# theislab/dca

Hardware: NVIDIA H100
Metric: cells/sec (ZINB AE epoch, device-timed) (higher is better)
Workload: dtype bf16-gemm/f32-acc/f32-loss

## Files before the change

dca_b200/csrc/dca_internal.cuh:

```cuda
#pragma once
#include <cuda_runtime.h>
#include <cuda_bf16.h>
#include <stdint.h>
#include <stddef.h>
#include <atomic>
#include "../../include/dca_b200.h"

namespace dca {

void set_error(const char* fmt, ...);
extern std::atomic<long long> g_launches;
inline void count_launch(int n = 1) { g_launches.fetch_add(n, std::memory_order_relaxed); }

#define DCA_CUDA_OK(expr)                                                              \
  do {                                                                                 \
    cudaError_t _e = (expr);                                                           \
    if (_e != cudaSuccess) {                                                           \
      ::dca::set_error("%s failed: %s (%s:%d)", #expr, cudaGetErrorString(_e), __FILE__, __LINE__); \
      return DCA_ERR_CUDA;                                                             \
    }                                                                                  \
  } while (0)

#define DCA_LAUNCH_CHECK()                                                             \
  do {                                                                                 \
// ... 42 lines not shown
int bn_train_finalize(const double* sum, const double* sq, int M, int N, float eps, float momentum,
                      float* mean, float* inv_std, float* moving_mean, float* moving_var, cudaStream_t s);
int bn_relu_fwd(const float* a, int64_t ld, int M, int N, const float* mean, const float* inv_std,
                const float* beta, float* xhat, float* h, __nv_bfloat16* h_bf16, cudaStream_t s);
int bn_infer_prepare(const float* moving_mean, const float* moving_var, int N, float eps,
                     float* mean, float* inv_std, cudaStream_t s);
int bias_relu_fwd(const float* a, int64_t ld, int M, int N, float* h, __nv_bfloat16* h_bf16, cudaStream_t s);
int relu_bwd(float* dh, const float* h, int64_t ld, int M, int N, cudaStream_t s);
int bn_bwd_apply(float* g_inout, const float* xhat, int64_t ld, int M, int N, const float* inv_std,
                 const double* sum_g, const double* sum_gx, float* dbeta, cudaStream_t s, int stat_rows = 0);
int col_sum_to_float(const double* sum, int N, float* out, cudaStream_t s);
int theta_prepare(const float* theta_raw, int G, float* theta, float* chain, cudaStream_t s);
int theta_grad_finish(const float* dtheta, const float* chain, int G, float scale, float* grad_out, cudaStream_t s);
int add_reg_grad(const float* w, float* g, int64_t n, float l1, float l2, cudaStream_t s);
int reg_penalty(const float* w, int64_t n, float l1, float l2, double* acc, cudaStream_t s);
int rmsprop_update(float* params, const float* grads, float* rms, int64_t n, float lr, float clip,
                   float rho, float eps, float grad_scale, __nv_bfloat16* shadow, float* loss_out, cudaStream_t s);
struct OptScalars { int kind; float lr, clip, gs, c0, c1, c2, c3, c4; };
int optimizer_update(float* params, const float* grads, float* s1, float* s2, int64_t n, OptScalars o, __nv_bfloat16* shadow,
                     float* loss_out, cudaStream_t s);
int glorot_fill(float* w, int64_t n, int fan_in, int fan_out, uint64_t seed, uint64_t stream_id, cudaStream_t s);
int fill_value(float* p, int64_t n, float v, cudaStream_t s);
int cast_to_bf16(const float* in, __nv_bfloat16* out, int64_t n, cudaStream_t s);

__device__ __forceinline__ float pre_log_value(float y, double sf64, int flags) {
  float q = (flags & DCA_PRE_SIZE_FACTORS) ? (float)((double)y / sf64) : y;
  if ((flags & DCA_PRE_LOG1P) && q != 0.f) q = (float)log1p((double)q);
  return q;
}
struct ExactXform {
  const double* n_counts; double median; int flags;
  const double* mean; const double* std; const float* x_zero;
};
int exact_zero_inputs(const double* mean, const double* std, int n, float* x_zero, cudaStream_t s);
int expand_counts(const void* cnt, int bits, const float* sf_in, int M, int n, const float* mean, const float* inv_std, int use_sf,
                  int use_log1p, float* Yout, void* Xout, int x_bf16, float* sf_out, const int64_t* ovf_indptr,
                  const void* ovf_entries, cudaStream_t s, const ExactXform* ex = nullptr, const int32_t* rows = nullptr);
int expand_sparse(const void* bitmap, const int64_t* nib_indptr, const void* nibbles, const float* sf_in, int M, int n,
                  const float* mean, const float* inv_std, int use_sf, int use_log1p, float* Yout, void* Xout, int x_bf16,
                  float* sf_out, const int64_t* ovf_indptr, const void* ovf_entries, int max_row_nibble_bytes, cudaStream_t s,
                  const ExactXform* ex = nullptr, const int32_t* rows = nullptr);
int check_packed_counts(const char* who, const dca_packed_counts* p);
int gather_rows_bf16(const void* X, int x_bf16, int64_t ldx, const int32_t* rows, int M, int n, __nv_bfloat16* out,
                     cudaStream_t s);

namespace tc {
int heads_fwd_tc(const __nv_bfloat16* Hb, int B, const __nv_bfloat16* const W[3], const float* const bias[3], int G,
                 int n_heads, const int kind[3], const float* row_scale, float* const out[3], int64_t ld_out, int sm_count,
                 cudaStream_t s);
int gene_gemm_tc(int mode, const __nv_bfloat16* const Z[3], int64_t ldz, const int32_t* rows, int B, int G, int n_heads,
                 const __nv_bfloat16* H, const __nv_bfloat16* const W[3], float* out_b, float* const dW[3], int64_t dW_ld,
                 int dW_transposed, float* const db[3], void* ws, size_t ws_bytes, int sm_count, cudaStream_t s);
size_t gene_gemm_workspace_bytes(int B);
int flash_zinb_tc(const __nv_bfloat16* H3, int B, int G, const __nv_bfloat16* const W[3], const float* const bias[3],
                  const float* Y, int64_t ldy, const int32_t* rows, const float* sf, float ridge, float inv_n,
                  float* dH3, float* const dW[3], float* const db[3], void* ws, size_t ws_bytes, double* loss_sum,
                  const double* penalty, float* loss_slot, double* epoch_acc, int batch, const float* lf_dev, int sm_count,
                  cudaStream_t s);
}

struct LossArgs {
  const float* Y; int64_t ldy; const int32_t* rows; const float* sf;
  const float* m; const float* d; const float* pi; int64_t ld;
  int B, G; int ae_type; float ridge; float inv_n;
  void* dzm; void* dzd; void* dzp; int grad_bf16;
  float* dtheta;
  double* loss_sum;
  void* ws; size_t ws_bytes;
  int counter_ready = 0;
  float* fin_loss_slot = nullptr; double* fin_epoch_acc = nullptr; const double* fin_penalty = nullptr; int fin_batch = 0;
};
size_t loss_workspace_bytes(int B, int G);
extern int g_fused_heads_default;
const float* loss_log_fact_table();
int zinb_loss_fwd_bwd(const LossArgs& a, cudaStream_t s);
int zinb_loss_fwd(const LossArgs& a, cudaStream_t s);

struct HeadsLossArgs {
  const __nv_bfloat16* H3; int B, G;
  const __nv_bfloat16* W[3]; const float* bias[3];
  const float* Y; int64_t ldy; const int32_t* rows; const float* sf;
  float ridge, inv_n;
  __nv_bfloat16* dz[3]; int64_t ldz;
  double* loss_sum; void* ws; size_t ws_bytes;
  int counter_ready = 0;
  float* fin_loss_slot = nullptr; double* fin_epoch_acc = nullptr; const double* fin_penalty = nullptr; int fin_batch = 0;
};
int heads_loss_tc(const HeadsLossArgs& a, cudaStream_t s);

}
```

dca_b200/csrc/engine.cu:

```cuda
#include <cmath>
#include <cstdarg>
#include <cstdio>
#include <cstring>
#include <cstdlib>
#include <string>
#include <vector>
#include "dca_internal.cuh"
#include "engine.h"

namespace dca {

std::atomic<long long> g_launches{0};
static thread_local char g_err[512] = "";

void set_error(const char* fmt, ...) {
  va_list ap;
  va_start(ap, fmt);
  vsnprintf(g_err, sizeof(g_err), fmt, ap);
  va_end(ap);
}

namespace {

inline size_t align_up(size_t v, size_t a = 256) { return (v + a - 1) / a * a; }
// ... 190 lines not shown
    cudaEvent_t e;
    if (cudaEventCreate(&e) != cudaSuccess) return;
    prof.ev.push_back(e); prof.phase.push_back(-1);
  }
  prof.phase[prof.n] = phase;
  cudaEventRecord(prof.ev[prof.n], s);
  ++prof.n;
}

int Engine::prof_collect() {
  if (prof.n == 0) return DCA_OK;
  DCA_CUDA_OK(cudaEventSynchronize(prof.ev[prof.n - 1]));
  for (size_t i = 0; i + 1 < prof.n; ++i) {
    const int ph = prof.phase[i];
    if (ph < 0 || ph >= DCA_N_PHASES) continue;
    float ms = 0.f;
    if (cudaEventElapsedTime(&ms, prof.ev[i], prof.ev[i + 1]) == cudaSuccess) { prof.ms[ph] += ms; prof.cnt[ph] += 1; }
  }
  prof.n = 0;
  return DCA_OK;
}

void Engine::bind(void* base_) {
  base = reinterpret_cast<char*>(base_);
}

int Engine::gemm_auto(GemmArgs g, cudaStream_t s) {
  const long long tiles = (long long)cdiv(g.M, 64) * cdiv(g.N, 64), target = 2ll * sm_count;
  int splits = 1;
  if (g.epilogue == EPI_ACCUM && tiles < target && g.K >= 256) {
    splits = (int)((target + tiles - 1) / tiles);
    const int maxs = g.K / 128;
    if (splits > maxs) splits = maxs;
    if (splits < 1) splits = 1;
  }
  g.splits = splits;
  return gemm_generic(g, s);
}

int Engine::forward(const void* X, int64_t ldx, const int32_t* rows, int Bn, bool training, cudaStream_t s) {
  const void* hin = X; int64_t ldin = ldx; int in_bf16 = x_override_bf16 ? 1 : (cfg.x_dtype == DCA_BF16); const int32_t* gather = rows;
  cur_x = XOperand{};
  if (tc_enc && (reinterpret_cast<uintptr_t>(X) & 15) == 0) {
    if (in_bf16 && ldx % 8 == 0) cur_x = XOperand{reinterpret_cast<const __nv_bfloat16*>(X), ldx, rows};
    else if (!in_bf16 && ldx % 4 == 0) {
      DCA_TRY(gather_rows_bf16(X, in_bf16, ldx, rows, Bn, cfg.n_in, bf(o_xb), s));
      cur_x = XOperand{bf(o_xb), cfg.n_in, nullptr};
    }
  }
  const bool fused = use_mid(Bn);
  for (int i = 0; i < (fused ? 1 : L); ++i) {
    Layer& l = lay[i];
    float* a = f(l.o_a);
    DCA_TRY(fill_rows_with_bias(a, l.out, Bn, l.out, pp(l.b), s));
    if (i == 0 && cur_x.base) {
      const __nv_bfloat16* Z[3] = {cur_x.base, cur_x.base, cur_x.base};
      const __nv_bfloat16* W1[3] = {bf(o_pbf) + lay[0].W, bf(o_pbf) + lay[0].W, bf(o_pbf) + lay[0].W};
      DCA_TRY(tc::gene_gemm_tc(1, Z, cur_x.ld, cur_x.rows, Bn, cfg.n_in, 1, nullptr, W1, a, nullptr, 0, 0, nullptr, base + o_ggws, ggws_bytes, sm_count, s));
    } else {
    GemmArgs g{};
    g.A = hin; g.lda = ldin; g.a_bf16 = in_bf16; g.transA = 0; g.a_rows = gather;
    g.B = pp(l.W); g.ldb = l.out; g.transB = 0;
    g.C = a; g.ldc = l.out; g.M = Bn; g.N = l.out; g.K = l.in; g.epilogue = EPI_ACCUM;
    DCA_TRY(gemm_auto(g, s));
    }
    if (fused) break;
    if (cfg.batchnorm) {
      if (training) {
        DCA_TRY(col_sums(a, nullptr, l.out, Bn, l.out, d(o_dsum), d(o_dprod), d(o_scratch), s));
        DCA_TRY(bn_allreduce(d(o_dsum), d(o_dprod), l.out, s));
        DCA_TRY(bn_train_finalize(d(o_dsum), d(o_dprod), bn_rows(Bn), l.out, cfg.bn_eps, cfg.bn_momentum, f(l.o_mean),
                                  f(l.o_inv), st(l.mm), st(l.mv), s));
      } else {
        DCA_TRY(bn_infer_prepare(st(l.mm), st(l.mv), l.out, cfg.bn_eps, f(l.o_mean), f(l.o_inv), s));
      }
    }
    DCA_TRY(act_fwd(l, Bn, training, (tc_heads && i == L - 1) ? bf(o_h3b) : nullptr, s));
    hin = f(l.o_h); ldin = l.out; in_bf16 = 0; gather = nullptr;
  }
  if (fused) {
    mid::Params mp;
    mid_params(mp, Bn, training);
    DCA_TRY(mid_forward(mp, s));
    hin = f(lay[L - 1].o_h); ldin = lay[L - 1].out; in_bf16 = 0; gather = nullptr;
  }
  head_in = hin; head_ld = ldin; head_bf16 = in_bf16; head_rows = gather;
  return DCA_OK;
}

int Engine::x_gather_sf(const float* sf, const int32_t* rows, int Bn, cudaStream_t s) {
  gather_sf_kernel<<<cdiv(Bn, 256), 256, 0, s>>>(sf, rows, Bn, f(o_sfb));
  DCA_LAUNCH_CHECK();
  return DCA_OK;
}

void Engine::mid_params(mid::Params& p, int Bn, bool training) {
  memset(&p, 0, sizeof(p));
  p.L = L; p.B = Bn; p.training = training ? 1 : 0; p.batchnorm = cfg.batchnorm; p.center = L / 2;
  for (int i = 0; i < L; ++i) {
    Layer& l = lay[i];
    p.w[i] = l.out; p.W[i] = pp(l.W); p.b[i] = pp(l.b);
    p.beta[i] = cfg.batchnorm ? pp(l.beta) : nullptr;
    p.mm[i] = cfg.batchnorm ? st(l.mm) : nullptr; p.mv[i] = cfg.batchnorm ? st(l.mv) : nullptr;
    p.mean[i] = f(l.o_mean); p.inv[i] = f(l.o_inv); p.xhat[i] = f(l.o_xhat); p.h[i] = f(l.o_h);
    p.gW[i] = gp(l.W); p.gb[i] = gp(l.b); p.gbeta[i] = cfg.batchnorm ? gp(l.beta) : nullptr;
  }
  p.a0 = f(lay[0].o_a); p.a_center = f(lay[L / 2].o_a);
  p.h_last_bf16 = tc_heads ? bf(o_h3b) : nullptr;
  p.partial = d(o_midpart); p.gpart = f(o_midgpart); p.bar = reinterpret_cast<unsigned*>(base + o_bar);
  p.eps = cfg.bn_eps; p.momentum = cfg.bn_momentum;
}

int Engine::heads_forward(int Bn, float* m_out, float* d_out, float* p_out, int64_t ld_out, const float* row_scale,
                          cudaStream_t s) {
  const int G = cfg.n_out;
  if (tc_heads && (ld_out % 4 == 0)) {
    float* outs_by_head[3] = {m_out, d_out, p_out};
    bool all = true;
    for (int k = 0; k < n_slots; ++k) all = all && outs_by_head[slot_head[k]] && ((reinterpret_cast<uintptr_t>(outs_by_head[slot_head[k]]) & 15) == 0);
    if (all) {
      float* outs[3] = {nullptr, nullptr, nullptr};
      for (int k = 0; k < n_slots; ++k) outs[k] = outs_by_head[slot_head[k]];
      for (int k = n_slots; k < 3; ++k) outs[k] = outs[0];
      const __nv_bfloat16* Wk[3]; const float* bk[3];
      for (int k = 0; k < 3; ++k) { const int kk = k < n_slots ? k : 0; Wk[k] = bf(o_pbf) + head_W[slot_head[kk]]; bk[k] = pp(head_b[slot_head[kk]]); }
      return tc::heads_fwd_tc(bf(o_h3b), Bn, Wk, bk, G, n_slots, slot_kind, row_scale, outs, ld_out, sm_count, s);
    }
  }
  struct H { int k; float* out; int epi; const float* rs; } hs[3] = {
      {0, m_out, EPI_MEAN_ACT, row_scale}, {1, d_out, EPI_DISP_ACT, nullptr}, {2, p_out, EPI_SIGMOID, nullptr}};
  for (auto& h : hs) {
    if (head_W[h.k] < 0 || !h.out) continue;
    GemmArgs g{};
    g.A = head_in; g.lda = head_ld; g.a_bf16 = head_bf16; g.transA = 0; g.a_rows = head_rows;
    g.B = pp(head_W[h.k]); g.ldb = G; g.transB = 0;
// ... 1094 lines not shown
```

dca_b200/csrc/gene_gemm_tc.cu:

```cuda
#include "engine.h"
#include "tc_common.cuh"

namespace dca {
namespace tc {
int g_gg_profile = 0;
int g_head_bwd_banded = 1;
int g_head_bwd_stagger = 1300;
namespace gg {

constexpr int kThreads = 256;
constexpr uint32_t kZBytes = 128 * 128 * 2;
constexpr uint32_t kWBytes = 64 * 128 * 2;
constexpr uint32_t kHBytes = 128 * 64 * 2;
constexpr uint32_t kOutBytes = 128 * 64 * 4;
constexpr uint32_t kOnesBytes = 16 * 128;
constexpr int kMaxGb = 4;
constexpr int kMaxSlots = 16;

static_assert(kWBytes == kHBytes, "the two item kinds of the banded launch share one stage shape");
template <bool DO_A, bool DO_B, bool BANDED>
constexpr int stages() { return DO_A && DO_B && !BANDED ? 2 : 3; }
template <bool DO_A, bool DO_B, bool BANDED>
constexpr uint32_t stage_bytes() { return BANDED ? kZBytes + kWBytes : kZBytes + (DO_B ? kWBytes : 0) + (DO_A ? kHBytes : 0); }
template <bool DO_A, bool DO_B, bool COLSUM, bool BANDED>
constexpr uint32_t smem_bytes() {
  return stages<DO_A, DO_B, BANDED>() * stage_bytes<DO_A, DO_B, BANDED>() + (DO_A ? kOutBytes : 0) + (COLSUM ? kOnesBytes : 0) + 1024;
}

struct BandItem { int kind, head, gr, gb0, ng, cb0, ncb; };

__host__ __device__ inline BandItem band_item(int k, int n_gb, int n_cb, int gpr, int ranges) {
  const int per_head = n_gb + ranges * n_cb, full_band = gpr + n_cb;
  BandItem it;
  it.head = k / per_head; k -= it.head * per_head;
  it.gr = min(k / full_band, ranges - 1); k -= it.gr * full_band;
  const int gb0 = it.gr * gpr, ng = min(n_gb, gb0 + gpr) - gb0, m = min(ng, n_cb);
  int idx;
  if (k < 2 * m) { it.kind = k & 1; idx = k >> 1; }
  else { it.kind = ng > n_cb ? 0 : 1; idx = k - m; }
  if (it.kind == 0) { it.gb0 = gb0 + idx; it.ng = 1; it.cb0 = 0; it.ncb = n_cb; }
  else { it.gb0 = gb0; it.ng = ng; it.cb0 = idx; it.ncb = 1; }
  return it;
}

struct Params {
  int B, G, n_heads;
  int n_cb, n_gb;
  int gb_per_item, cb_per_item;
  int gene_ranges, cell_splits;
  int total_items;
  int stagger;
  float* db[3];
  float* part; int64_t part_stride;
  const int32_t* rows; const __nv_bfloat16* zsrc; int64_t ldz;
};

__device__ __forceinline__ void cp_async_16(uint32_t smem_dst, const void* src, uint32_t src_bytes) {
  asm volatile("cp.async.cg.shared.global [%0], [%1], 16, %2;" ::"r"(smem_dst), "l"(src), "r"(src_bytes) : "memory");
}
__device__ __forceinline__ void cp_async_commit() { asm volatile("cp.async.commit_group;" ::: "memory"); }
template <int N>
__device__ __forceinline__ void cp_async_wait() { asm volatile("cp.async.wait_group %0;" ::"n"(N) : "memory"); }

template <bool DO_A, bool DO_B, bool COLSUM, bool WK, int MAXG, bool BANDED>
__global__ void __launch_bounds__(kThreads, 1)
gene_gemm_kernel(const __grid_constant__ CUtensorMap map_z0, const __grid_constant__ CUtensorMap map_z1,
                 const __grid_constant__ CUtensorMap map_z2, const __grid_constant__ CUtensorMap map_h,
                 const __grid_constant__ CUtensorMap map_w0, const __grid_constant__ CUtensorMap map_w1,
                 const __grid_constant__ CUtensorMap map_w2, const __grid_constant__ CUtensorMap map_dw0, const __grid_constant__ CUtensorMap map_dw1,
                 const __grid_constant__ CUtensorMap map_dw2, const int dw_transposed, const Params p) {
  static_assert(!BANDED || (DO_A && DO_B && MAXG == 1), "banded items hold one gene block of (a) accumulators");
  constexpr int kStages = stages<DO_A, DO_B, BANDED>();
  constexpr uint32_t kStage = stage_bytes<DO_A, DO_B, BANDED>();
  constexpr uint32_t kHOff = kZBytes + (DO_B && !BANDED ? kWBytes : 0);
  extern __shared__ __align__(1024) uint8_t smem_raw[];
  uint8_t* smem = smem_raw + ((1024u - (smem_u32(smem_raw) & 1023u)) & 1023u);
  uint8_t* s_st = smem;
  float* s_o = reinterpret_cast<float*>(s_st + kStages * kStage);
  uint8_t* s_ones = reinterpret_cast<uint8_t*>(s_o) + (DO_A ? kOutBytes : 0);
  __shared__ uint64_t full[kStages];

  if (threadIdx.x == 0) {
    for (int i = 0; i < kStages; ++i) mbar_init(&full[i], 1);
    fence_barrier_init();
  }
  if (COLSUM) {
    for (int i = threadIdx.x; i < (int)kOnesBytes / 4; i += kThreads) reinterpret_cast<uint32_t*>(s_ones)[i] = 0x3F803F80u;
    fence_proxy_async_smem();
  }
  __syncthreads();

  const int wg = threadIdx.x >> 7, w = (threadIdx.x >> 5) & 3, l = threadIdx.x & 31;
  const int frow = 16 * w + (l >> 2), fcol = 2 * (l & 3);

  auto stage_begin = [&]() {
    if (threadIdx.x == 0) bulk_wait_read<0>();
    __syncthreads();
  };
  auto stage_end = [&](const CUtensorMap* m, int c0, int c1) {
    fence_proxy_async_smem();
    __syncthreads();
    if (threadIdx.x == 0) { tma_reduce_add_2d(m, c0, c1, s_o); bulk_commit(); }
  };

  uint32_t T0 = 0;
  const bool gather = p.rows != nullptr;
  const int g_rh = threadIdx.x >> 3, g_c = threadIdx.x & 7, g_h = g_rh & 1, g_r0 = g_rh >> 1;
  const uint32_t g_dst = g_h * (kZBytes / 2) + g_r0 * 128 + ((g_c ^ (g_r0 & 7)) << 4);
  int src_row[8];
  if constexpr (BANDED) {
    if (p.stagger > 0 && blockIdx.x < p.total_items) {
      const BandItem it = band_item(blockIdx.x, p.n_gb, p.n_cb, p.gb_per_item, p.gene_ranges);
      const long long wait = (long long)(it.kind ? it.cb0 : it.gb0 - it.gr * p.gb_per_item) * p.stagger;
      if (threadIdx.x == 0) {
        const long long c0 = clock64();
        while (clock64() - c0 < wait) __nanosleep(100);
      }
      __syncthreads();
    }
  }
  for (int item = blockIdx.x; item < p.total_items; item += gridDim.x) {
    int head, gr, gb0, ng, cb0, ncb;
    bool ia = DO_A, ib = DO_B;
    if constexpr (BANDED) {
      const BandItem it = band_item(item, p.n_gb, p.n_cb, p.gb_per_item, p.gene_ranges);
// ... 162 lines not shown
            const int g = gb * 128 + wg * 64 + frow;
            if (g < p.G) atomicAdd(dbh + g, acc_c[j][0]);
            if (g + 8 < p.G) atomicAdd(dbh + g + 8, acc_c[j][2]);
          }
        }
      }
    }
  }
  if (threadIdx.x == 0) bulk_wait<0>();
}

__global__ void gene_gemm_reduce_kernel(const float* __restrict__ part, int slots, int64_t stride, float* __restrict__ out,
                                        int64_t n) {
  const int64_t i = ((int64_t)blockIdx.x * blockDim.x + threadIdx.x) * 4;
  if (i >= n) return;
  float4 acc = *reinterpret_cast<const float4*>(out + i);
  for (int sl = 0; sl < slots; ++sl) {
    const float4 v = __ldcs(reinterpret_cast<const float4*>(part + sl * stride + i));
    acc.x += v.x; acc.y += v.y; acc.z += v.z; acc.w += v.w;
  }
  *reinterpret_cast<float4*>(out + i) = acc;
}

void plan_a(Params& p, int n_heads, int sm_count) {
  int best_gpi = 1; long long best_cost = -1;
  for (int gpi = 1; gpi <= kMaxGb; ++gpi) {
    const long long items = (long long)cdiv(p.n_gb, gpi) * n_heads, rounds = (items + sm_count - 1) / sm_count;
    const long long cost = rounds * ((long long)gpi * p.n_cb + 2ll * gpi);
    if (best_cost < 0 || cost < best_cost) { best_cost = cost; best_gpi = gpi; }
  }
  p.gb_per_item = best_gpi; p.gene_ranges = cdiv(p.n_gb, best_gpi);
  p.cb_per_item = p.n_cb; p.cell_splits = 1;
  p.total_items = p.gene_ranges * n_heads;
}
void plan_b(Params& p, int n_heads, int sm_count) {
  p.cb_per_item = 1; p.cell_splits = p.n_cb;
  int gsplits = cdiv(4 * sm_count, p.n_cb * n_heads); if (gsplits < 1) gsplits = 1;
  if (gsplits > kMaxSlots / n_heads) gsplits = kMaxSlots / n_heads;
  if (gsplits > p.n_gb) gsplits = p.n_gb;
  while (gsplits > 1 && cdiv(p.n_gb, gsplits) < 4) --gsplits;
  p.gb_per_item = cdiv(p.n_gb, gsplits); p.gene_ranges = cdiv(p.n_gb, p.gb_per_item);
  p.total_items = p.gene_ranges * p.cell_splits * n_heads;
}
void plan_banded(Params& p, int n_heads, int sm_count, int* grid) {
  plan_b(p, n_heads, sm_count);
  p.total_items = n_heads * (p.n_gb + p.gene_ranges * p.n_cb);
  const int band = p.gb_per_item + p.n_cb;
  *grid = min(p.total_items, sm_count >= band ? sm_count / band * band : sm_count);
}

}

size_t gene_gemm_workspace_bytes(int B) { return sizeof(float) * (size_t)gg::kMaxSlots * cdiv(B, 128) * 128 * 64; }

int gene_gemm_tc(int mode, const __nv_bfloat16* const Z[3], int64_t ldz, const int32_t* rows, int B, int G, int n_heads,
                 const __nv_bfloat16* H, const __nv_bfloat16* const W[3], float* out_b, float* const dW[3], int64_t dW_ld,
                 int dW_transposed, float* const db[3], void* ws, size_t ws_bytes, int sm_count, cudaStream_t s) {
  using namespace gg;
  if (ldz % 8 != 0) { set_error("gene_gemm_tc: ldz must be a multiple of 8 (16-byte TMA stride)"); return DCA_ERR_BAD_ARG; }
  if (mode < 1 || mode > 3) { set_error("gene_gemm_tc: bad mode %d", mode); return DCA_ERR_BAD_ARG; }
  if (rows && (mode == 3 || n_heads != 1)) { set_error("gene_gemm_tc: row indices are for modes 1 and 2 (one Z)"); return DCA_ERR_BAD_ARG; }
  const bool do_a = mode & 2, do_b = mode & 1;
  if (do_b && (!ws || ws_bytes < gene_gemm_workspace_bytes(B))) { set_error("gene_gemm_tc: workspace too small"); return DCA_ERR_BAD_ARG; }
  CUtensorMap mz[3], mh, mw[3], mdw[3];
  for (int i = 0; i < 3; ++i) DCA_TRY(make_tensor_map_2d(&mz[i], Z[i < n_heads ? i : 0], 2, 1, (uint64_t)B, (uint64_t)G, (uint64_t)ldz, 128, 64, 1));
  mh = mz[0];
  for (int i = 0; i < 3; ++i) mw[i] = mdw[i] = mz[0];
  if (do_a) {
    DCA_TRY(make_tensor_map_2d(&mh, H, 2, 1, (uint64_t)B, 64, 64, 128, 64, 1));
    for (int i = 0; i < 3; ++i) {
      float* d = dW[i < n_heads ? i : 0];
      if (dW_transposed) DCA_TRY(make_tensor_map_2d(&mdw[i], d, 4, 0, 64, (uint64_t)G, (uint64_t)dW_ld, 64, 128, 0));
      else {
        if (dW_ld != 64) { set_error("gene_gemm_tc: non-transposed dW needs ld == 64"); return DCA_ERR_BAD_ARG; }
        DCA_TRY(make_tensor_map_2d(&mdw[i], d, 4, 0, (uint64_t)G, 64, 64, 128, 64, 0));
      }
    }
  }
  if (do_b) {
    for (int i = 0; i < 3; ++i) {
      const __nv_bfloat16* w = W[i < n_heads ? i : 0];
      if (mode == 3) DCA_TRY(make_tensor_map_2d(&mw[i], w, 2, 1, 64, (uint64_t)G, (uint64_t)G, 64, 64, 1));
      else DCA_TRY(make_tensor_map_2d(&mw[i], w, 2, 1, (uint64_t)G, 64, 64, 128, 64, 1));
    }
  }
  Params base{};
  base.B = B; base.G = G; base.n_heads = n_heads;
  base.n_cb = cdiv(B, 128); base.n_gb = cdiv(G, 128);
  for (int i = 0; i < 3; ++i) base.db[i] = db ? db[i] : nullptr;
  base.part = reinterpret_cast<float*>(ws); base.part_stride = (int64_t)base.n_cb * 128 * 64;
  base.rows = rows; base.zsrc = Z[0]; base.ldz = ldz;

#define DCA_GG_LAUNCH(P, GRID, A, Bb, Cc, WKk, MG, BND)                                                                \
  do {                                                                                                                 \
    static bool attr = false;                                                                                          \
    constexpr uint32_t sm = smem_bytes<A, Bb, Cc, BND>();                                                              \
    if (!attr) { DCA_CUDA_OK(cudaFuncSetAttribute(gene_gemm_kernel<A, Bb, Cc, WKk, MG, BND>, cudaFuncAttributeMaxDynamicSharedMemorySize, (int)sm)); attr = true; } \
    gene_gemm_kernel<A, Bb, Cc, WKk, MG, BND><<<GRID, kThreads, sm, s>>>(mz[0], mz[1], mz[2], mh, mw[0], mw[1], mw[2],  \
                                                                          mdw[0], mdw[1], mdw[2], dW_transposed, P);  \
    DCA_LAUNCH_CHECK();                                                                                                \
  } while (0)

  if (mode == 3 && g_head_bwd_banded) {
    Params p = base;
    int grid = 0;
    plan_banded(p, n_heads, sm_count, &grid);
    p.stagger = g_head_bwd_stagger;
    DCA_GG_LAUNCH(p, grid, true, true, true, true, 1, true);
    const int64_t n = (int64_t)B * 64;
    gene_gemm_reduce_kernel<<<(unsigned)cdiv(n / 4, 256), 256, 0, s>>>(p.part, p.gene_ranges * n_heads, p.part_stride, out_b, n);
    DCA_LAUNCH_CHECK();
    return DCA_OK;
  }
  if (do_a) {
    Params p = base;
    plan_a(p, n_heads, sm_count);
    const int grid = min(p.total_items, sm_count);
    if (mode == 3) DCA_GG_LAUNCH(p, grid, true, false, true, false, kMaxGb, false);
    else DCA_GG_LAUNCH(p, grid, true, false, false, false, kMaxGb, false);
  }
  if (do_b) {
    Params p = base;
    plan_b(p, n_heads, sm_count);
    const int grid = min(p.total_items, sm_count);
    if (mode == 3) DCA_GG_LAUNCH(p, grid, false, true, false, true, 1, false);
    else DCA_GG_LAUNCH(p, grid, false, true, false, false, 1, false);
    const int64_t n = (int64_t)B * 64;
    gene_gemm_reduce_kernel<<<(unsigned)cdiv(n / 4, 256), 256, 0, s>>>(p.part, p.gene_ranges * n_heads, p.part_stride, out_b, n);
    DCA_LAUNCH_CHECK();
  }
#undef DCA_GG_LAUNCH
  return DCA_OK;
}

}
}

using namespace dca;
extern "C" int dca_tc_gene_gemm_rows(int32_t mode, const void* Z0, const void* Z1, const void* Z2, int64_t ldz,
                                     const int32_t* rows, int32_t batch, int32_t genes, int32_t n_heads, const void* H,
                                     const void* W, float* out_b, float* dW0, float* dW1, float* dW2, int64_t dW_ld,
                                     int32_t dW_transposed, float* db0, float* db1, float* db2, void* stream, int32_t sm_count) {
  if (!Z0 || batch <= 0 || genes <= 0 || n_heads < 1 || n_heads > 3) { set_error("dca_tc_gene_gemm: bad argument"); return DCA_ERR_BAD_ARG; }
  int dev = 0, sms = 132;
  cudaGetDevice(&dev);
  cudaDeviceGetAttribute(&sms, cudaDevAttrMultiProcessorCount, dev);
  if (sm_count > 0 && sm_count < sms) sms = sm_count;
  const __nv_bfloat16* Z[3] = {(const __nv_bfloat16*)Z0, (const __nv_bfloat16*)Z1, (const __nv_bfloat16*)Z2};
  float* dW[3] = {dW0, dW1, dW2};
  float* db[3] = {db0, db1, db2};
  const __nv_bfloat16* Wp[3];
  for (int i = 0; i < 3; ++i) Wp[i] = (const __nv_bfloat16*)W + (mode == 3 ? (size_t)(i < n_heads ? i : 0) * 64 * genes : 0);
  cudaStream_t st = (cudaStream_t)stream;
  const size_t ws_bytes = tc::gene_gemm_workspace_bytes(batch);
  void* ws = nullptr;
  DCA_CUDA_OK(cudaMallocAsync(&ws, ws_bytes, st));
  const int rc = tc::gene_gemm_tc(mode, Z, ldz, rows, batch, genes, n_heads, (const __nv_bfloat16*)H, Wp, out_b, dW,
                                  dW_ld, dW_transposed, db, ws, ws_bytes, sms, st);
  DCA_CUDA_OK(cudaFreeAsync(ws, st));
  return rc;
}
extern "C" int dca_tc_gene_gemm_sms(int32_t mode, const void* Z0, const void* Z1, const void* Z2, int64_t ldz,
                                    int32_t batch, int32_t genes, int32_t n_heads, const void* H, const void* W, float* out_b,
                                    float* dW0, float* dW1, float* dW2, int64_t dW_ld, int32_t dW_transposed, float* db0,
                                    float* db1, float* db2, void* stream, int32_t sm_count) {
  return dca_tc_gene_gemm_rows(mode, Z0, Z1, Z2, ldz, nullptr, batch, genes, n_heads, H, W, out_b, dW0, dW1, dW2, dW_ld,
                               dW_transposed, db0, db1, db2, stream, sm_count);
}
extern "C" int dca_tc_gene_gemm(int32_t mode, const void* Z0, const void* Z1, const void* Z2, int64_t ldz, int32_t batch,
                                int32_t genes, int32_t n_heads, const void* H, const void* W, float* out_b, float* dW0,
                                float* dW1, float* dW2, int64_t dW_ld, int32_t dW_transposed, float* db0, float* db1,
                                float* db2, void* stream) {
  return dca_tc_gene_gemm_sms(mode, Z0, Z1, Z2, ldz, batch, genes, n_heads, H, W, out_b, dW0, dW1, dW2, dW_ld,
                              dW_transposed, db0, db1, db2, stream, 0);
}
extern "C" int dca_head_bwd_schedule(int32_t batch, int32_t genes, int32_t n_heads, int32_t sm_count, int32_t banded,
                                     int32_t* items, int64_t cap, int64_t* n_items, int32_t* grid) {
  if (batch <= 0 || genes <= 0 || n_heads < 1 || n_heads > 3 || sm_count < 1 || !n_items || !grid) {
    set_error("dca_head_bwd_schedule: bad argument"); return DCA_ERR_BAD_ARG;
// ... 38 lines not shown
```

dca_b200/csrc/mid_stack.cu:

```cuda
#include "dca_internal.cuh"
#include "mid_stack.h"
#include <cstdio>
#include <cstdlib>

namespace dca {
namespace mid {

constexpr int kThreads = 256;
#define MID_STAMP(i) do { if (p.dbg && blockIdx.x == 0 && threadIdx.x == 0) p.dbg[i] = clock64(); } while (0)
constexpr int kGenWord = 32;
constexpr int kStripStride = kMaxW + 4;
typedef float Strip[kStripStride];
typedef float WRow[kMaxW + 1];

__device__ __forceinline__ void grid_barrier(unsigned* bar, unsigned n, unsigned& gen) {
  __syncthreads();
  if (threadIdx.x == 0) {
    asm volatile("fence.acq_rel.gpu;" ::: "memory");
    const unsigned arrived = atomicAdd(&bar[0], 1u);
    if (arrived == n - 1) {
      bar[0] = 0;
      asm volatile("fence.acq_rel.gpu;" ::: "memory");
      atomicAdd(&bar[kGenWord], 1u);
    } else {
// ... 60 lines not shown
    for (int i = 0; i < kPairsPerWarp; ++i) tot[warp + i * (kThreads / 32)] = x[i][0];
  }
  __syncthreads();
}

__device__ __forceinline__ void strip_gemm(Strip* in, WRow* Ws, const float* bias, int rows, int w_in, int w_out, Strip* out) {
  const int c = threadIdx.x & 63, g = threadIdx.x >> 6;
  if (c < w_out) {
    const float bv = bias ? bias[c] : 0.f;
    for (int r0 = g * 4; r0 < rows; r0 += 16) {
      float acc[4] = {0.f, 0.f, 0.f, 0.f};
#pragma unroll 4
      for (int k = 0; k < w_in; k += 4) {
        const float w0 = Ws[k][c], w1 = Ws[k + 1][c], w2 = Ws[k + 2][c], w3 = Ws[k + 3][c];
#pragma unroll
        for (int j = 0; j < 4; ++j) {
          const float4 x = *reinterpret_cast<const float4*>(&in[r0 + j][k]);
          acc[j] = fmaf(x.x, w0, fmaf(x.y, w1, fmaf(x.z, w2, fmaf(x.w, w3, acc[j]))));
        }
      }
#pragma unroll
      for (int j = 0; j < 4; ++j)
        if (r0 + j < rows) out[r0 + j][c] = acc[j] + bv;
    }
  }
}

constexpr size_t kStripFloats = (size_t)(kMaxRows + 4) * kStripStride;
constexpr size_t kWsFloats = (size_t)kMaxW * (kMaxW + 1);
constexpr int kWSlots = DCA_MAX_HIDDEN - 1;
constexpr size_t kSmemBytes = sizeof(double) * (8 * kMaxW + 2 * kMaxW) + sizeof(float) * (2 * kStripFloats + kWSlots * kWsFloats + 2 * kMaxW) + 16;

__global__ void __launch_bounds__(kThreads, 1) mid_forward_kernel(const Params p) {
  extern __shared__ __align__(16) unsigned char smem_mid[];
  double (*red)[kMaxW] = reinterpret_cast<double (*)[kMaxW]>(smem_mid);
  double* tot = reinterpret_cast<double*>(smem_mid) + 8 * kMaxW;
  float* fbase = reinterpret_cast<float*>(tot + 2 * kMaxW);
  Strip* cur = reinterpret_cast<Strip*>(fbase);
  Strip* nxt = reinterpret_cast<Strip*>(fbase + kStripFloats);
  WRow* Ws = reinterpret_cast<WRow*>(fbase + 2 * kStripFloats);
  float* s_mean = fbase + 2 * kStripFloats + kWSlots * kWsFloats;
  float* s_inv = s_mean + kMaxW;
  __shared__ unsigned s_gen;
  if (threadIdx.x == 0) s_gen = *reinterpret_cast<volatile unsigned*>(&p.bar[kGenWord]);
  __syncthreads();
  unsigned gen = s_gen;
  MID_STAMP(0);

  const int row0 = blockIdx.x * p.rows_per_cta;
  const int rows = max(0, min(p.rows_per_cta, p.B - row0));
  for (int i = threadIdx.x; i < (int)kStripFloats; i += kThreads) { (&cur[0][0])[i] = 0.f; (&nxt[0][0])[i] = 0.f; }
  __syncthreads();
  const int tc = threadIdx.x & 63, tr = threadIdx.x >> 6;
  constexpr int kRowIters = kMaxRows / 4, kKIters = kMaxW / 4;
  float a0r[kRowIters];
#pragma unroll
  for (int i = 0; i < kRowIters; ++i) {
    const int r = tr + 4 * i;
    a0r[i] = (tc < p.w[0] && r < rows) ? p.a0[(size_t)(row0 + r) * p.w[0] + tc] : 0.f;
  }
  for (int l0 = 1; l0 < p.L; l0 += 2) {
    float wr[2][kKIters];
#pragma unroll
    for (int d = 0; d < 2; ++d) {
      const int l = l0 + d;
      const int win = l < p.L ? p.w[l - 1] : 0, w = l < p.L ? p.w[l] : 0;
#pragma unroll
      for (int i = 0; i < kKIters; ++i) { const int k = tr + 4 * i; wr[d][i] = (k < win && tc < w) ? p.W[l][(size_t)k * w + tc] : 0.f; }
    }
#pragma unroll
    for (int d = 0; d < 2; ++d) {
      if (l0 + d >= p.L) break;
      WRow* Wl = Ws + (size_t)(l0 + d - 1) * kMaxW;
#pragma unroll
      for (int i = 0; i < kKIters; ++i) Wl[tr + 4 * i][tc] = wr[d][i];
    }
  }
  float mm_old[DCA_MAX_HIDDEN], mv_old[DCA_MAX_HIDDEN];
#pragma unroll
  for (int l = 0; l < DCA_MAX_HIDDEN; ++l) {
    const bool mine = p.batchnorm && p.training && blockIdx.x == 0 && l < p.L && (int)threadIdx.x < p.w[l];
    mm_old[l] = mine ? p.mm[l][threadIdx.x] : 0.f; mv_old[l] = mine ? p.mv[l][threadIdx.x] : 0.f;
  }
  float beta_r[DCA_MAX_HIDDEN];
#pragma unroll
  for (int l = 0; l < DCA_MAX_HIDDEN; ++l) beta_r[l] = (p.batchnorm && l < p.L && tc < p.w[l]) ? p.beta[l][tc] : 0.f;
  if (tc < p.w[0]) {
#pragma unroll
    for (int i = 0; i < kRowIters; ++i) { const int r = tr + 4 * i; if (r < rows) cur[r][tc] = a0r[i]; }
  }
  __syncthreads();
  MID_STAMP(1);
  Strip* a = cur;
  Strip* o = nxt;
  for (int l = 0; l < p.L; ++l) {
    const int w = p.w[l];
    if (l > 0) {
      const int win = p.w[l - 1];
      strip_gemm(a, Ws + (size_t)(l - 1) * kMaxW, p.b[l], rows, win, w, o);
      __syncthreads();
      Strip* t = a; a = o; o = t;
      MID_STAMP(2 + l * 5);
    }
    if (l == p.center && p.a_center && !(l == 0 && p.a_center == p.a0) && tc < w)
      for (int r = tr; r < rows; r += 4) p.a_center[(size_t)(row0 + r) * w + tc] = a[r][tc];
    if (p.batchnorm) {
      if (p.training) {
        double* part = p.partial + (size_t)(l & 1) * kMaxCtas * 2 * kMaxW;
        cta_col_sums(a, a, rows, w, part + blockIdx.x, red);
        MID_STAMP(3 + l * 5);
        grid_barrier(p.bar, gridDim.x, gen);
        MID_STAMP(4 + l * 5);
        fold_partials(part, gridDim.x, w, tot);
        MID_STAMP(5 + l * 5);
        if (threadIdx.x < w) {
          const int c = threadIdx.x;
          const double inv_b = 1.0 / (double)p.B;
          const double mu = tot[c] * inv_b;
          double var = tot[kMaxW + c] * inv_b - mu * mu;
          if (var < 0.0) var = 0.0;
          s_mean[c] = (float)mu;
          const float vf = (float)(var + (double)p.eps);
          float r = rsqrtf(vf);
          r = r * (1.5f - 0.5f * vf * r * r);
          s_inv[c] = r;
          if (blockIdx.x == 0) {
            p.mean[l][c] = s_mean[c]; p.inv[l][c] = r;
#pragma unroll
            for (int q = 0; q < DCA_MAX_HIDDEN; ++q)
              if (q == l) {
                p.mm[l][c] = p.momentum * mm_old[q] + (1.0f - p.momentum) * (float)mu;
                p.mv[l][c] = p.momentum * mv_old[q] + (1.0f - p.momentum) * (float)var;
              }
          }
        }
        __syncthreads();
      } else {
        if (threadIdx.x < w) { s_mean[threadIdx.x] = p.mm[l][threadIdx.x]; s_inv[threadIdx.x] = rsqrtf(p.mv[l][threadIdx.x] + p.eps); }
        __syncthreads();
      }
    }
    const bool last = (l == p.L - 1);
    if (tc < w) {
      const float mean_c = p.batchnorm ? s_mean[tc] : 0.f, inv_c = p.batchnorm ? s_inv[tc] : 1.f;
      float beta_c = 0.f;
#pragma unroll
      for (int q = 0; q < DCA_MAX_HIDDEN; ++q) if (q == l) beta_c = beta_r[q];
      for (int r = tr; r < rows; r += 4) {
        const size_t gi = (size_t)(row0 + r) * w + tc;
        float v = a[r][tc];
        if (p.batchnorm) {
          const float xh = (v - mean_c) * inv_c;
          if (p.training) p.xhat[l][gi] = xh;
          v = xh + beta_c;
        }
        v = fmaxf(v, 0.f);
        a[r][tc] = v;
// ... 129 lines not shown
            s[2] = fmaf(hv[j].z, gv[j], s[2]); s[3] = fmaf(hv[j].w, gv[j], s[3]);
          }
        }
        if (k0 == tr * 4) MID_STAMP(25 + (p.L - 1 - l) * 3);
#pragma unroll
        for (int j = 0; j < 4; ++j)
          if (k0 + j < win) gpart_l[(size_t)(kMaxW + (k0 + j) * w + tc) * kMaxCtas] = s[j];
        if (k0 == tr * 4) MID_STAMP(26 + (p.L - 1 - l) * 3);
      }
    __syncthreads();
    MID_STAMP(7 + (p.L - 1 - l) * 8);
    constexpr int kRowGroups = kMaxRows / 16;
    float dhv[kRowGroups][4];
    if (tc < win) {
#pragma unroll
      for (int q = 0; q < kRowGroups; ++q) {
        const int r0 = tr * 4 + q * 16;
        float acc[4] = {0.f, 0.f, 0.f, 0.f};
        if (r0 < rows)
#pragma unroll 4
          for (int c = 0; c < w; c += 4) {
            const float w0 = Ws[tc][c], w1 = Ws[tc][c + 1], w2 = Ws[tc][c + 2], w3 = Ws[tc][c + 3];
#pragma unroll
            for (int j = 0; j < 4; ++j) {
              const float4 x = *reinterpret_cast<const float4*>(&g[r0 + j][c]);
              acc[j] = fmaf(x.x, w0, fmaf(x.y, w1, fmaf(x.z, w2, fmaf(x.w, w3, acc[j]))));
            }
          }
#pragma unroll
        for (int j = 0; j < 4; ++j) dhv[q][j] = acc[j];
      }
    }
    __syncthreads();
    if (tc < win) {
#pragma unroll
      for (int q = 0; q < kRowGroups; ++q)
#pragma unroll
        for (int j = 0; j < 4; ++j) { const int r = tr * 4 + q * 16 + j; if (r < rows) xh[r][tc] = dhv[q][j]; }
    }
    __syncthreads();
    for (int i = threadIdx.x; i < (int)kStripFloats; i += kThreads) (&g[0][0])[i] = 0.f;
    __syncthreads();
    if (tc < win)
      for (int r = tr; r < rows; r += 4) g[r][tc] = xh[r][tc];
    __syncthreads();
    MID_STAMP(8 + (p.L - 1 - l) * 8);
  }
  grid_barrier(p.bar, gridDim.x, gen);
  for (int e = blockIdx.x * kThreads + threadIdx.x; e < p.L * kGradSlots; e += gridDim.x * kThreads) {
    const int l = e / kGradSlots, o = e % kGradSlots, w = p.w[l];
    float* dst;
    if (o < kMaxW) { if (o >= w) continue; dst = p.gb[l] + o; }
    else { if (l == 0 || o - kMaxW >= p.w[l - 1] * w) continue; dst = p.gW[l] + (o - kMaxW); }
    const float* src = p.gpart + (size_t)e * kMaxCtas;
    float sum = 0.f;
    for (int c = 0; c < (int)gridDim.x; ++c) sum += __ldcg(src + c);
    *dst += sum;
  }
  MID_STAMP(31);
}

}

bool mid_supported(const int* widths, int L) {
  if (L < 1) return false;
  for (int i = 0; i < L; ++i) if (widths[i] > mid::kMaxW) return false;
  return true;
}

static int mid_fill(mid::Params& p, int B) {
  static const int rows_target = [] { const char* e = getenv("DCA_MID_ROWS"); int v = e ? atoi(e) : 32; return (v >= 16 && v <= mid::kMaxRows) ? v : 32; }();
  int ctas = cdiv(B, rows_target);
  if (ctas > mid::kMaxCtas) ctas = mid::kMaxCtas;
  if (p.max_ctas > 0 && ctas > p.max_ctas) { ctas = p.max_ctas; if ((long long)ctas * mid::kMaxRows < B) ctas = cdiv(B, mid::kMaxRows); }
  if ((long long)ctas * mid::kMaxRows < B) { set_error("mid_stack: batch %d exceeds %d rows", B, mid::kMaxRows * mid::kMaxCtas); return DCA_ERR_UNSUPPORTED; }
  int rpc = cdiv(B, ctas);
  if (rpc < 16) rpc = 16;
  rpc = (rpc + 3) & ~3;
  if (rpc > mid::kMaxRows) rpc = mid::kMaxRows;
  while ((long long)rpc * mid::kMaxCtas < B) rpc += 4;
  p.rows_per_cta = rpc; p.n_ctas = cdiv(B, rpc);
  return DCA_OK;
}

size_t mid_partial_doubles() { return (size_t)2 * mid::kMaxCtas * 2 * mid::kMaxW; }
size_t mid_grad_partial_floats(int L) { return (size_t)L * mid::kGradSlots * mid::kMaxCtas; }

static int mid_attr() {
  static bool done = false;
  if (!done) {
    DCA_CUDA_OK(cudaFuncSetAttribute(mid::mid_forward_kernel, cudaFuncAttributeMaxDynamicSharedMemorySize, (int)mid::kSmemBytes));
    DCA_CUDA_OK(cudaFuncSetAttribute(mid::mid_backward_kernel, cudaFuncAttributeMaxDynamicSharedMemorySize, (int)mid::kSmemBytes));
    done = true;
  }
  return DCA_OK;
}

bool mid_device_ok() {
  static thread_local int ok_dev = -1, ok = 0;
  int dev = 0;
  if (cudaGetDevice(&dev) != cudaSuccess) { (void)cudaGetLastError(); return false; }
  if (ok_dev == dev) return ok != 0;
  ok_dev = dev; ok = 0;
  if (mid_attr() != DCA_OK) return false;
  int coop = 0, sms = 0, nf = 0, nb = 0;
  if (cudaDeviceGetAttribute(&coop, cudaDevAttrCooperativeLaunch, dev) != cudaSuccess || !coop) return false;
  if (cudaDeviceGetAttribute(&sms, cudaDevAttrMultiProcessorCount, dev) != cudaSuccess) return false;
  if (cudaOccupancyMaxActiveBlocksPerMultiprocessor(&nf, mid::mid_forward_kernel, mid::kThreads, mid::kSmemBytes) != cudaSuccess) return false;
  if (cudaOccupancyMaxActiveBlocksPerMultiprocessor(&nb, mid::mid_backward_kernel, mid::kThreads, mid::kSmemBytes) != cudaSuccess) return false;
// ... 53 lines not shown
```

dca_b200/csrc/mid_stack.h:

```cpp
#pragma once
#include "dca_internal.cuh"

namespace dca {
namespace mid {

constexpr int kMaxW = 64;
constexpr int kMaxCtas = 128;
constexpr int kMaxRows = 64;
constexpr int kGradSlots = kMaxW + kMaxW * kMaxW;

struct Params {
  int L, B, training, batchnorm, center, rows_per_cta, n_ctas;
  int max_ctas;
  int w[DCA_MAX_HIDDEN];
  const float* W[DCA_MAX_HIDDEN];
  const float* b[DCA_MAX_HIDDEN];
  const float* beta[DCA_MAX_HIDDEN];
  float* mm[DCA_MAX_HIDDEN]; float* mv[DCA_MAX_HIDDEN];
  float* mean[DCA_MAX_HIDDEN]; float* inv[DCA_MAX_HIDDEN];
  float* xhat[DCA_MAX_HIDDEN]; float* h[DCA_MAX_HIDDEN];
  float* a0;
  float* a_center;
  __nv_bfloat16* h_last_bf16;
  float* dh_last;
  float* gW[DCA_MAX_HIDDEN]; float* gb[DCA_MAX_HIDDEN]; float* gbeta[DCA_MAX_HIDDEN];
  float* da0; __nv_bfloat16* da0_bf16;
  double* partial;
  float* gpart;
  unsigned* bar;
  float eps, momentum;
  long long* dbg;
};

}

bool mid_supported(const int* widths, int L);
bool mid_device_ok();
size_t mid_partial_doubles();
size_t mid_grad_partial_floats(int L);
int mid_forward(mid::Params& p, cudaStream_t s);
int mid_backward(mid::Params& p, cudaStream_t s);

}
```

Baseline: 3.113 million.

## Fuse first-layer split-K partial reduction and bias into the mid-stack kernel

When the fused mid-stack runs, the first-layer gene GEMM no longer launches its reduce kernel or fills the output with bias. The mid-stack forward kernel sums the per-slot split partials plus bias directly into its shared strip, which removes one launch, the bias fill, and an extra global round trip of the a0 activation. The change also adjusts the pipeline stage counts for the non-colsum gene GEMM variants and vectorises the gradient partial reduction with unrolled float4 loads. Risks are more register pressure in the mid kernel and more shared memory from extra stages. The a_center write path is altered so that layer 0 is still recorded when a0 is no longer materialised.

```diff
diff --git a/dca_b200/csrc/dca_internal.cuh b/dca_b200/csrc/dca_internal.cuh
--- a/dca_b200/csrc/dca_internal.cuh
+++ b/dca_b200/csrc/dca_internal.cuh
@@ -118,6 +118,7 @@
                  const __nv_bfloat16* H, const __nv_bfloat16* const W[3], float* out_b, float* const dW[3], int64_t dW_ld,
                  int dW_transposed, float* const db[3], void* ws, size_t ws_bytes, int sm_count, cudaStream_t s);
 size_t gene_gemm_workspace_bytes(int B);
+int gene_gemm_slots(int B, int G, int n_heads, int sm_count);
 int flash_zinb_tc(const __nv_bfloat16* H3, int B, int G, const __nv_bfloat16* const W[3], const float* const bias[3],
                   const float* Y, int64_t ldy, const int32_t* rows, const float* sf, float ridge, float inv_n,
                   float* dH3, float* const dW[3], float* const db[3], void* ws, size_t ws_bytes, double* loss_sum,
diff --git a/dca_b200/csrc/engine.cu b/dca_b200/csrc/engine.cu
--- a/dca_b200/csrc/engine.cu
+++ b/dca_b200/csrc/engine.cu
@@ -266,11 +266,13 @@
   for (int i = 0; i < (fused ? 1 : L); ++i) {
     Layer& l = lay[i];
     float* a = f(l.o_a);
-    DCA_TRY(fill_rows_with_bias(a, l.out, Bn, l.out, pp(l.b), s));
+    const bool slots = fused && i == 0 && cur_x.base;
+    if (!slots) DCA_TRY(fill_rows_with_bias(a, l.out, Bn, l.out, pp(l.b), s));
     if (i == 0 && cur_x.base) {
       const __nv_bfloat16* Z[3] = {cur_x.base, cur_x.base, cur_x.base};
       const __nv_bfloat16* W1[3] = {bf(o_pbf) + lay[0].W, bf(o_pbf) + lay[0].W, bf(o_pbf) + lay[0].W};
-      DCA_TRY(tc::gene_gemm_tc(1, Z, cur_x.ld, cur_x.rows, Bn, cfg.n_in, 1, nullptr, W1, a, nullptr, 0, 0, nullptr, base + o_ggws, ggws_bytes, sm_count, s));
+      DCA_TRY(tc::gene_gemm_tc(1, Z, cur_x.ld, cur_x.rows, Bn, cfg.n_in, 1, nullptr, W1, slots ? nullptr : a, nullptr, 0, 0,
+                               nullptr, base + o_ggws, ggws_bytes, sm_count, s));
     } else {
     GemmArgs g{};
     g.A = hin; g.lda = ldin; g.a_bf16 = in_bf16; g.transA = 0; g.a_rows = gather;
@@ -295,6 +297,11 @@
   if (fused) {
     mid::Params mp;
     mid_params(mp, Bn, training);
+    if (cur_x.base) {
+      mp.a0_part = reinterpret_cast<const float*>(base + o_ggws);
+      mp.a0_slots = tc::gene_gemm_slots(Bn, cfg.n_in, 1, sm_count);
+      mp.a0_stride = (int64_t)cdiv(Bn, 128) * 128 * 64;
+    }
     DCA_TRY(mid_forward(mp, s));
     hin = f(lay[L - 1].o_h); ldin = lay[L - 1].out; in_bf16 = 0; gather = nullptr;
   }
diff --git a/dca_b200/csrc/gene_gemm_tc.cu b/dca_b200/csrc/gene_gemm_tc.cu
--- a/dca_b200/csrc/gene_gemm_tc.cu
+++ b/dca_b200/csrc/gene_gemm_tc.cu
@@ -18,13 +18,13 @@
 constexpr int kMaxSlots = 16;
 
 static_assert(kWBytes == kHBytes, "the two item kinds of the banded launch share one stage shape");
-template <bool DO_A, bool DO_B, bool BANDED>
-constexpr int stages() { return DO_A && DO_B && !BANDED ? 2 : 3; }
+template <bool DO_A, bool DO_B, bool COLSUM, bool BANDED>
+constexpr int stages() { return DO_A && DO_B ? (BANDED ? 3 : 2) : (COLSUM ? 3 : 4); }
 template <bool DO_A, bool DO_B, bool BANDED>
 constexpr uint32_t stage_bytes() { return BANDED ? kZBytes + kWBytes : kZBytes + (DO_B ? kWBytes : 0) + (DO_A ? kHBytes : 0); }
 template <bool DO_A, bool DO_B, bool COLSUM, bool BANDED>
 constexpr uint32_t smem_bytes() {
-  return stages<DO_A, DO_B, BANDED>() * stage_bytes<DO_A, DO_B, BANDED>() + (DO_A ? kOutBytes : 0) + (COLSUM ? kOnesBytes : 0) + 1024;
+  return stages<DO_A, DO_B, COLSUM, BANDED>() * stage_bytes<DO_A, DO_B, BANDED>() + (DO_A ? kOutBytes : 0) + (COLSUM ? kOnesBytes : 0) + 1024;
 }
 
 struct BandItem { int kind, head, gr, gb0, ng, cb0, ncb; };
@@ -70,7 +70,7 @@
                  const __grid_constant__ CUtensorMap map_w2, const __grid_constant__ CUtensorMap map_dw0, const __grid_constant__ CUtensorMap map_dw1,
                  const __grid_constant__ CUtensorMap map_dw2, const int dw_transposed, const Params p) {
   static_assert(!BANDED || (DO_A && DO_B && MAXG == 1), "banded items hold one gene block of (a) accumulators");
-  constexpr int kStages = stages<DO_A, DO_B, BANDED>();
+  constexpr int kStages = stages<DO_A, DO_B, COLSUM, BANDED>();
   constexpr uint32_t kStage = stage_bytes<DO_A, DO_B, BANDED>();
   constexpr uint32_t kHOff = kZBytes + (DO_B && !BANDED ? kWBytes : 0);
   extern __shared__ __align__(1024) uint8_t smem_raw[];
@@ -339,6 +339,12 @@
 }
 
 size_t gene_gemm_workspace_bytes(int B) { return sizeof(float) * (size_t)gg::kMaxSlots * cdiv(B, 128) * 128 * 64; }
+int gene_gemm_slots(int B, int G, int n_heads, int sm_count) {
+  gg::Params p{};
+  p.n_cb = cdiv(B, 128); p.n_gb = cdiv(G, 128);
+  gg::plan_b(p, n_heads, sm_count);
+  return p.gene_ranges * n_heads;
+}
 
 int gene_gemm_tc(int mode, const __nv_bfloat16* const Z[3], int64_t ldz, const int32_t* rows, int B, int G, int n_heads,
                  const __nv_bfloat16* H, const __nv_bfloat16* const W[3], float* out_b, float* const dW[3], int64_t dW_ld,
@@ -412,6 +418,7 @@
     const int grid = min(p.total_items, sm_count);
     if (mode == 3) DCA_GG_LAUNCH(p, grid, false, true, false, true, 1, false);
     else DCA_GG_LAUNCH(p, grid, false, true, false, false, 1, false);
+    if (!out_b) return DCA_OK;
     const int64_t n = (int64_t)B * 64;
     gene_gemm_reduce_kernel<<<(unsigned)cdiv(n / 4, 256), 256, 0, s>>>(p.part, p.gene_ranges * n_heads, p.part_stride, out_b, n);
     DCA_LAUNCH_CHECK();
diff --git a/dca_b200/csrc/mid_stack.cu b/dca_b200/csrc/mid_stack.cu
--- a/dca_b200/csrc/mid_stack.cu
+++ b/dca_b200/csrc/mid_stack.cu
@@ -136,12 +136,38 @@
   for (int i = threadIdx.x; i < (int)kStripFloats; i += kThreads) { (&cur[0][0])[i] = 0.f; (&nxt[0][0])[i] = 0.f; }
   __syncthreads();
   const int tc = threadIdx.x & 63, tr = threadIdx.x >> 6;
-  constexpr int kRowIters = kMaxRows / 4, kKIters = kMaxW / 4;
+  constexpr int kRowIters = kMaxRows / 4, kKIters = kMaxW / 4, kSumIters = kMaxRows / 16;
   float a0r[kRowIters];
+  const int c4 = (threadIdx.x & 15) * 4, sr = threadIdx.x >> 4;
+  float4 a0s[kSumIters];
+  if (p.a0_part) {
+    const float4 bv = make_float4(p.b[0][c4], p.b[0][c4 + 1], p.b[0][c4 + 2], p.b[0][c4 + 3]);
+#pragma unroll
+    for (int i = 0; i < kSumIters; ++i) a0s[i] = bv;
+    for (int sl0 = 0; sl0 < p.a0_slots; sl0 += 4) {
+      float4 v[4][kSumIters];
+#pragma unroll
+      for (int j = 0; j < 4; ++j)
+#pragma unroll
+        for (int i = 0; i < kSumIters; ++i) {
+          const int r = sr + 16 * i;
+          v[j][i] = (sl0 + j < p.a0_slots && r < rows)
+                        ? __ldcs(reinterpret_cast<const float4*>(p.a0_part + (sl0 + j) * p.a0_stride + (size_t)(row0 + r) * 64 + c4))
+                        : make_float4(0.f, 0.f, 0.f, 0.f);
+        }
+#pragma unroll
+      for (int j = 0; j < 4; ++j)
+        if (sl0 + j < p.a0_slots)
+#pragma unroll
+          for (int i = 0; i < kSumIters; ++i) {
+            a0s[i].x += v[j][i].x; a0s[i].y += v[j][i].y; a0s[i].z += v[j][i].z; a0s[i].w += v[j][i].w;
+          }
+    }
+  }
 #pragma unroll
   for (int i = 0; i < kRowIters; ++i) {
     const int r = tr + 4 * i;
-    a0r[i] = (tc < p.w[0] && r < rows) ? p.a0[(size_t)(row0 + r) * p.w[0] + tc] : 0.f;
+    a0r[i] = (!p.a0_part && tc < p.w[0] && r < rows) ? p.a0[(size_t)(row0 + r) * p.w[0] + tc] : 0.f;
   }
   for (int l0 = 1; l0 < p.L; l0 += 2) {
     float wr[2][kKIters];
@@ -169,7 +195,10 @@
   float beta_r[DCA_MAX_HIDDEN];
 #pragma unroll
   for (int l = 0; l < DCA_MAX_HIDDEN; ++l) beta_r[l] = (p.batchnorm && l < p.L && tc < p.w[l]) ? p.beta[l][tc] : 0.f;
-  if (tc < p.w[0]) {
+  if (p.a0_part) {
+#pragma unroll
+    for (int i = 0; i < kSumIters; ++i) { const int r = sr + 16 * i; if (r < rows) *reinterpret_cast<float4*>(&cur[r][c4]) = a0s[i]; }
+  } else if (tc < p.w[0]) {
 #pragma unroll
     for (int i = 0; i < kRowIters; ++i) { const int r = tr + 4 * i; if (r < rows) cur[r][tc] = a0r[i]; }
   }
@@ -186,7 +215,7 @@
       Strip* t = a; a = o; o = t;
       MID_STAMP(2 + l * 5);
     }
-    if (l == p.center && p.a_center && !(l == 0 && p.a_center == p.a0) && tc < w)
+    if (l == p.center && p.a_center && !(l == 0 && p.a_center == p.a0 && !p.a0_part) && tc < w)
       for (int r = tr; r < rows; r += 4) p.a_center[(size_t)(row0 + r) * w + tc] = a[r][tc];
     if (p.batchnorm) {
       if (p.training) {
@@ -422,9 +451,18 @@
     float* dst;
     if (o < kMaxW) { if (o >= w) continue; dst = p.gb[l] + o; }
     else { if (l == 0 || o - kMaxW >= p.w[l - 1] * w) continue; dst = p.gW[l] + (o - kMaxW); }
-    const float* src = p.gpart + (size_t)e * kMaxCtas;
+    const float4* src = reinterpret_cast<const float4*>(p.gpart + (size_t)e * kMaxCtas);
+    float4 x[kMaxCtas / 4];
+#pragma unroll
+    for (int i = 0; i < kMaxCtas / 4; ++i) x[i] = __ldcg(src + i);
     float sum = 0.f;
-    for (int c = 0; c < (int)gridDim.x; ++c) sum += __ldcg(src + c);
+#pragma unroll
+    for (int i = 0; i < kMaxCtas / 4; ++i) {
+      if (4 * i < (int)gridDim.x) sum += x[i].x;
+      if (4 * i + 1 < (int)gridDim.x) sum += x[i].y;
+      if (4 * i + 2 < (int)gridDim.x) sum += x[i].z;
+      if (4 * i + 3 < (int)gridDim.x) sum += x[i].w;
+    }
     *dst += sum;
   }
   MID_STAMP(31);
diff --git a/dca_b200/csrc/mid_stack.h b/dca_b200/csrc/mid_stack.h
--- a/dca_b200/csrc/mid_stack.h
+++ b/dca_b200/csrc/mid_stack.h
@@ -20,6 +20,7 @@
   float* mean[DCA_MAX_HIDDEN]; float* inv[DCA_MAX_HIDDEN];
   float* xhat[DCA_MAX_HIDDEN]; float* h[DCA_MAX_HIDDEN];
   float* a0;
+  const float* a0_part; int a0_slots; int64_t a0_stride;
   float* a_center;
   __nv_bfloat16* h_last_bf16;
   float* dh_last;
```

Result: faster. 3.187 million, median of 6 (+2.4%).
